# xipengwang/AprilSAM

Hardware: NVIDIA H100
Metric: Gauss-Newton solves/sec (batch + incremental) on M3500 & 100k-pose graph (higher is better)
Workload: dtype f64

## Files before the change

### aprilsam_b200/csrc/asam_cuda.cu

```cuda

#include <cuda_runtime.h>

#include <cmath>
#include <cstdarg>
#include <cstdint>
#include <cstdio>
#include <cstdlib>
#include <cstring>
#include <ctime>

#include "asam_cuda.h"

#define ASAM_EXPORT extern "C" __attribute__((visibility("default")))

static thread_local char g_err[512] = "";

static int set_err(const char *fmt, ...)
{
    va_list ap;
    va_start(ap, fmt);
    vsnprintf(g_err, sizeof(g_err), fmt, ap);
    va_end(ap);
    return 1;
}
// ... 527 lines not shown
        const int v = atoi(getenv("ASAM_DIAG_MMA")) != 0;
        CK(cudaMemcpyToSymbol(g_diag_mma, &v, sizeof(int)));
    }
    if (getenv("ASAM_DMAP_AHEAD")) {
        const int v = atoi(getenv("ASAM_DMAP_AHEAD")) != 0;
        CK(cudaMemcpyToSymbol(g_dmap_ahead, &v, sizeof(int)));
    }
    if (getenv("ASAM_PF_GROUPS")) {
        const int v = atoi(getenv("ASAM_PF_GROUPS")) != 0;
        CK(cudaMemcpyToSymbol(g_pf_groups, &v, sizeof(int)));
    }
    if (getenv("ASAM_KEEP"))
        d->keep_off = atoi(getenv("ASAM_KEEP")) == 0;
    if (getenv("ASAM_TILE_MODE"))
        d->tile_mode = atoi(getenv("ASAM_TILE_MODE"));
    if (getenv("ASAM_SMALL_STEP"))
        d->small_ok = atoi(getenv("ASAM_SMALL_STEP")) != 0;
    memset(d->pin_down, 0, 64);
    *out = d;
    return 0;
}

ASAM_EXPORT void asam_dev_destroy(asam_dev_t *d)
{
    if (!d)
        return;
    cudaSetDevice(d->device);
    cudaStreamSynchronize(d->stream);
    Buf *all[] = { &d->f_type, &d->f_a, &d->f_b, &d->f_z, &d->f_W, &d->f_slot, &d->lp, &d->st, &d->node2q, &d->q2node,
                   &d->Adiag, &d->Aoff, &d->Bq, &d->y, &d->x, &d->dinv, &d->sn, &d->ipool, &d->arena, &d->arrive,
                   &d->xdone, &d->xblk, &d->tbar, &d->tasks_full, &d->nwait_full, &d->btasks_full, &d->tasks_tmp, &d->nwait_tmp,
                   &d->btasks_tmp, &d->keep_tmp, &d->leaf_tasks, &d->top_tasks, &d->top_nwait, &d->ctrl, &d->partial, &d->patch_ids, &d->patch_desc, &d->pts, &d->flush, &d->trace_fac, &d->trace_bs, &d->ptrace };
    for (int i = 0; i < 2; i++)
        if (d->tev[i])
            cudaEventDestroy(d->tev[i]);
    for (Buf *b : all)
        if (b->p)
            cudaFree(b->p);
    if (d->pin)
        cudaFreeHost(d->pin);
    if (d->pin_down)
        cudaFreeHost(d->pin_down);
    if (d->dstage)
        cudaFree(d->dstage);
    if (d->up_ev)
        cudaEventDestroy(d->up_ev);
    free(d->items);
    free(d->pend);
    free(d->sh_owner); free(d->sh_q0); free(d->sh_qn); free(d->sh_off); free(d->sh_cnt);
    for (int i = 0; i < 6; i++)
        if (d->ev[i])
            cudaEventDestroy(d->ev[i]);
    cudaStreamDestroy(d->stream);
    delete d;
}

ASAM_EXPORT int asam_reserve(asam_dev_t *d, int n_nodes, int n_factors, int n_slots, int n_sn, int64_t ipool_ints,
                             int64_t arena_doubles)
{
    CK(cudaSetDevice(d->device));
    size_t N = (size_t) (n_nodes > 0 ? n_nodes : 0), Fn = (size_t) (n_factors > 0 ? n_factors : 0);
    size_t S = (size_t) (n_slots > 0 ? n_slots : 0), SN = (size_t) (n_sn > 0 ? n_sn : 0);
    int rc = 0;
    rc |= buf_reserve(d, d->f_type, Fn * sizeof(int), true, false);
    rc |= buf_reserve(d, d->f_a, Fn * sizeof(int), true, false);
    rc |= buf_reserve(d, d->f_b, Fn * sizeof(int), true, false);
    rc |= buf_reserve(d, d->f_slot, Fn * sizeof(int), true, false);
    rc |= buf_reserve(d, d->f_z, Fn * 3 * sizeof(double), true, false);
    rc |= buf_reserve(d, d->f_W, Fn * 9 * sizeof(double), true, false);
    rc |= buf_reserve(d, d->lp, N * 3 * sizeof(double), true, false);
    rc |= buf_reserve(d, d->st, N * 3 * sizeof(double), true, false);
    rc |= buf_reserve(d, d->node2q, N * sizeof(int), true, false);
    rc |= buf_reserve(d, d->q2node, N * sizeof(int), true, false);
    rc |= buf_reserve(d, d->Adiag, N * 9 * sizeof(double), true, true);
    rc |= buf_reserve(d, d->Bq, N * 3 * sizeof(double), true, true);
    rc |= buf_reserve(d, d->y, N * 3 * sizeof(double), true, true);
    rc |= buf_reserve(d, d->x, N * 3 * sizeof(double), true, true);
    rc |= buf_reserve(d, d->dinv, N * 3 * sizeof(double), true, true);
    rc |= buf_reserve(d, d->Aoff, S * 9 * sizeof(double), true, true);
    rc |= buf_reserve(d, d->sn, SN * sizeof(asam_sn_desc_t), true, false);
    rc |= buf_reserve(d, d->arrive, SN * sizeof(int), true, true);
    rc |= buf_reserve(d, d->xdone, SN * sizeof(int), true, true);
    rc |= buf_reserve(d, d->xblk, SN * sizeof(int), true, true);
    rc |= buf_reserve(d, d->tbar, 2 * SN * sizeof(int), true, true);
    rc |= buf_reserve(d, d->ipool, (size_t) ipool_ints * sizeof(int), true, false);
    rc |= buf_reserve(d, d->arena, (size_t) arena_doubles * sizeof(double), true, false);
    return rc;
}

ASAM_EXPORT int asam_upload_factors(asam_dev_t *d, int first, int count, const int32_t *type, const int32_t *na,
                                    const int32_t *nb, const double *z3, const double *W9)
{
    if (count <= 0)
        return 0;
    size_t need = (size_t) first + count;
    if (need * sizeof(int) > d->f_type.cap)
        return set_err("asam_upload_factors: capacity (call asam_reserve)");
    int rc = 0;
    rc |= upload(d, (int *) d->f_type.p + first, type, count * sizeof(int));
    rc |= upload(d, (int *) d->f_a.p + first, na, count * sizeof(int));
    rc |= upload(d, (int *) d->f_b.p + first, nb, count * sizeof(int));
    rc |= upload(d, (double *) d->f_z.p + 3 * (size_t) first, z3, count * 3 * sizeof(double));
    rc |= upload(d, (double *) d->f_W.p + 9 * (size_t) first, W9, count * 9 * sizeof(double));
    return rc;
}

ASAM_EXPORT int asam_upload_points(asam_dev_t *d, int which, int first, int count, const double *p3)
{
    if (count <= 0)
        return 0;
    Buf &b = which == 0 ? d->lp : d->st;
    if (((size_t) first + count) * 3 * sizeof(double) > b.cap)
        return set_err("asam_upload_points: capacity");
    return upload(d, (double *) b.p + 3 * (size_t) first, p3, (size_t) count * 3 * sizeof(double));
}

ASAM_EXPORT int asam_copy_points(asam_dev_t *d, int from, int to, int first, int count)
{
    if (count <= 0 || from == to)
        return 0;
    CK(cudaSetDevice(d->device));
    Buf &src = from == 0 ? d->lp : d->st, &dst = to == 0 ? d->lp : d->st;
    const size_t off = (size_t) first * 3 * sizeof(double), bytes = (size_t) count * 3 * sizeof(double);
    if (off + bytes > src.cap || off + bytes > dst.cap)
        return set_err("asam_copy_points: capacity");
    if (flush_uploads(d))
        return 1;
    CK(cudaMemcpyAsync((char *) dst.p + off, (const char *) src.p + off, bytes, cudaMemcpyDeviceToDevice, d->stream));
    return 0;
}

ASAM_EXPORT int asam_upload_node2q(asam_dev_t *d, int first, int count, const int32_t *node2q)
{
    if (count <= 0)
        return 0;
    if (((size_t) first + count) * sizeof(int) > d->node2q.cap)
        return set_err("asam_upload_node2q: capacity");
    return upload(d, (int *) d->node2q.p + first, node2q, (size_t) count * sizeof(int));
}

ASAM_EXPORT int asam_upload_q2node(asam_dev_t *d, int first, int count, const int32_t *q2node)
{
    if (count <= 0)
        return 0;
    if (((size_t) first + count) * sizeof(int) > d->q2node.cap)
        return set_err("asam_upload_q2node: capacity");
    return upload(d, (int *) d->q2node.p + first, q2node, (size_t) count * sizeof(int));
}

ASAM_EXPORT int asam_upload_fslot(asam_dev_t *d, int first, int count, const int32_t *fslot)
{
    if (count <= 0)
        return 0;
    if (((size_t) first + count) * sizeof(int) > d->f_slot.cap)
        return set_err("asam_upload_fslot: capacity");
    return upload(d, (int *) d->f_slot.p + first, fslot, (size_t) count * sizeof(int));
}

ASAM_EXPORT int asam_upload_ipool(asam_dev_t *d, int64_t first, int64_t count, const int32_t *data)
{
    if (count <= 0)
        return 0;
    if ((size_t) (first + count) * sizeof(int) > d->ipool.cap)
        return set_err("asam_upload_ipool: capacity");
    return upload(d, (int *) d->ipool.p + first, data, (size_t) count * sizeof(int));
}

// ... 852 lines not shown
```

### aprilsam_b200/csrc/asam_kernels.cuh

```cuda
#pragma once

#include <cuda_runtime.h>

#include <cstdint>

#include "asam_cuda.h"

#define ASAM_TR_FLAG (1 << 30)
#define ASAM_MAX_CACHED_CHILDREN 24

__device__ __forceinline__ double d_mod2pi(double v)
{
    const double twopi = 6.2831853071795862319959;
    const double pi = 3.141592653589793238462643383279502884196;
    double w = v + pi;
    return (w - twopi * floor(w / twopi)) - pi;
}

__device__ __forceinline__ void d_atb(const double *A, const double *B, double *C)
{
#pragma unroll
    for (int i = 0; i < 3; i++)
#pragma unroll
        for (int j = 0; j < 3; j++) {
// ... 525 lines not shown
                bulk_g2s(Lj + (size_t) p * ASAM_LDJ, col + (cb0 - shj), bj, bar);
            }
        }
        for (int e = tid; e < (pb4 - pb) * ASAM_LDI; e += nt)
            Li[(size_t) pb * ASAM_LDI + e] = 0.0;
        for (int e = tid; e < (pb4 - pb) * ASAM_LDJ; e += nt)
            Lj[(size_t) pb * ASAM_LDJ + e] = 0.0;
    } else {
        for (int p = warp; p < pb4; p += 2 * nwarps) {
            double vj[2][2], vi[2][8];
#pragma unroll
            for (int h = 0; h < 2; h++) {
                const int pp = p + h * nwarps;
                const double *src = F + (size_t) (k0 + min(pp, pb - 1)) * ld;
#pragma unroll
                for (int u = 0; u < 2; u++)
                    vj[h][u] = (pp < pb && lane + 32 * u < ncol) ? __ldcg(src + cb0 + lane + 32 * u) : 0.0;
#pragma unroll
                for (int u = 0; u < 8; u++)
                    vi[h][u] = (pp < pb && lane + 32 * u < nrow) ? __ldcg(src + rb0 + lane + 32 * u) : 0.0;
            }
#pragma unroll
            for (int h = 0; h < 2; h++) {
                const int pp = p + h * nwarps;
                if (pp < pb4) {
#pragma unroll
                    for (int u = 0; u < 2; u++)
                        Lj[lane + 32 * u + pp * ASAM_LDJ] = vj[h][u];
#pragma unroll
                    for (int u = 0; u < 8; u++)
                        Li[lane + 32 * u + pp * ASAM_LDI] = vi[h][u];
                }
            }
        }
    }
    const int g = lane >> 2, t = lane & 3;
    const int r0 = warp * 8 * MT;
    const int nnt = (ncol + 7) >> 3;
    const int rowmax = rb0 + min(r0 + 8 * MT, nrow) - 1;
    const int nneed = (r0 < nrow && rowmax >= cb0) ? min(nnt, ((rowmax - cb0) >> 3) + 1) : 0;
    double acc[MT][8][2];
#pragma unroll
    for (int mt = 0; mt < MT; mt++)
#pragma unroll
        for (int q = 0; q < 8; q++)
#pragma unroll
            for (int e = 0; e < 2; e++) {
                const int ii = r0 + 8 * mt + g, jj = 8 * q + 2 * t + e;
                const bool ok = q < nneed && ii < nrow && jj < ncol && rb0 + ii >= cb0 + jj;
                acc[mt][q][e] = ok ? __ldcg(&F[(rb0 + ii) + (size_t) (cb0 + jj) * ld]) : 0.0;
            }
    if (bulk) {
        mbar_wait(bar, parity);
        parity ^= 1u;
    }
    __syncthreads();
    if (nneed > 0) {
        const double *ai = Li + shi + r0 + g + (size_t) t * ASAM_LDI;
        const double *bj_ = Lj + shj + g + (size_t) t * ASAM_LDJ;
#pragma unroll 2
        for (int kk = 0; kk < pb4; kk += 4) {
            double av[MT];
#pragma unroll
            for (int mt = 0; mt < MT; mt++)
                av[mt] = -ai[8 * mt + (size_t) kk * ASAM_LDI];
#pragma unroll
            for (int q = 0; q < 8; q++) {
                if (q < nneed) {
                    const double bv = bj_[8 * q + (size_t) kk * ASAM_LDJ];
#pragma unroll
                    for (int mt = 0; mt < MT; mt++)
                        dmma_8x8x4(acc[mt][q][0], acc[mt][q][1], av[mt], bv);
                }
            }
        }
#pragma unroll
        for (int mt = 0; mt < MT; mt++)
#pragma unroll
            for (int q = 0; q < 8; q++)
#pragma unroll
                for (int e = 0; e < 2; e++) {
                    const int ii = r0 + 8 * mt + g, jj = 8 * q + 2 * t + e;
                    if (q < nneed && ii < nrow && jj < ncol && rb0 + ii >= cb0 + jj) {
                        F[(rb0 + ii) + (size_t) (cb0 + jj) * ld] = acc[mt][q][e];
                        if (Dout)
                            Dout[ii + jj * ASAM_TPB] = acc[mt][q][e];
                    }
                }
    }
}

#define ASAM_LDW 52
#define ASAM_WS_DOUBLES(m) (2 * (size_t) ((m) + 2) * ASAM_LDW)

template <int MT>
__device__ __noinline__ void tile_rm(double *F, const int ld, const double *Wk, const int pb4, const int cb0, const int ncol,
                                     const int rb0, const int nrow, const int out_mode, double *Out, double *Li, double *Lj,
                                     unsigned long long *bar, unsigned &parity)
{
    const int tid = threadIdx.x;
    const int lane = tid & 31, warp = tid >> 5;
    const bool same = rb0 == cb0 && nrow >= ncol;
    __syncthreads();
    if (warp == 0) {
        asm volatile("fence.proxy.async;" ::: "memory");
        if (lane == 0) {
            const unsigned bi = (unsigned) nrow * ASAM_LDW * 8u, bj = same ? 0u : (unsigned) ncol * ASAM_LDW * 8u;
            mbar_expect_tx(bar, bi + bj);
            bulk_g2s(Li, Wk + (size_t) rb0 * ASAM_LDW, bi, bar);
            if (!same)
                bulk_g2s(Lj, Wk + (size_t) cb0 * ASAM_LDW, bj, bar);
        }
    }
    const double *Ljs = same ? Li : Lj;
    const int g = lane >> 2, t = lane & 3;
    const int r0 = warp * 8 * MT;
    const int nnt = (ncol + 7) >> 3;
    const int rowmax = rb0 + min(r0 + 8 * MT, nrow) - 1;
    const int nneed = (r0 < nrow && rowmax >= cb0) ? min(nnt, ((rowmax - cb0) >> 3) + 1) : 0;
    double acc[MT][8][2];
#pragma unroll
    for (int mt = 0; mt < MT; mt++)
#pragma unroll
        for (int q = 0; q < 8; q++)
#pragma unroll
            for (int e = 0; e < 2; e++) {
                const int ii = r0 + 8 * mt + g, jj = 8 * q + 2 * t + e;
                const bool ok = q < nneed && ii < nrow && jj < ncol && rb0 + ii >= cb0 + jj;
                acc[mt][q][e] = ok ? __ldcg(&F[(rb0 + ii) + (size_t) (cb0 + jj) * ld]) : 0.0;
            }
    mbar_wait(bar, parity);
    parity ^= 1u;
    if (nneed > 0) {
        const double *ai = Li + (size_t) (r0 + g) * ASAM_LDW + t;
        const double *bj_ = Ljs + (size_t) g * ASAM_LDW + t;
#pragma unroll 2
        for (int kk = 0; kk < pb4; kk += 4) {
            double av[MT];
#pragma unroll
            for (int mt = 0; mt < MT; mt++)
                av[mt] = -ai[(size_t) (8 * mt) * ASAM_LDW + kk];
#pragma unroll
            for (int q = 0; q < 8; q++) {
                if (q < nneed) {
                    const double bv = bj_[(size_t) (8 * q) * ASAM_LDW + kk];
#pragma unroll
                    for (int mt = 0; mt < MT; mt++)
                        dmma_8x8x4(acc[mt][q][0], acc[mt][q][1], av[mt], bv);
                }
            }
        }
    }
    if (out_mode == 2)
        __syncthreads();
    if (nneed > 0) {
#pragma unroll
        for (int mt = 0; mt < MT; mt++)
#pragma unroll
            for (int q = 0; q < 8; q++)
#pragma unroll
                for (int e = 0; e < 2; e++) {
                    const int ii = r0 + 8 * mt + g, jj = 8 * q + 2 * t + e;
                    if (q < nneed && ii < nrow && jj < ncol && rb0 + ii >= cb0 + jj) {
                        if (out_mode == 0)
                            F[(rb0 + ii) + (size_t) (cb0 + jj) * ld] = acc[mt][q][e];
                        else if (out_mode == 1)
                            Out[ii + jj * ASAM_TPB] = acc[mt][q][e];
                        else
                            Out[ii + jj * ASAM_TROWS] = acc[mt][q][e];
                    }
                }
    }
}

struct TeamCtx {
    int *tbar_s;
    int G, w, phase;
    long long spin_limit;
    int *err;
    int sn;
};

__device__ __forceinline__ bool team_barrier(TeamCtx &tc, int *s_flag)
{
    __syncthreads();
    if (threadIdx.x == 0) {
        red_release_add(tc.tbar_s, 1);
        const int target = (++tc.phase) * tc.G;
        SpinClock spins;
        int ok = 1;
        while (ld_volatile(tc.tbar_s) < target) {
            __nanosleep(20);
            if (spin_over(spins, tc.spin_limit) || ld_volatile(tc.err) < 0) {
                atomicCAS(tc.err, 0, -(1 + tc.sn));
                ok = 0;
                break;
            }
        }
        ld_acquire(tc.tbar_s);
        *s_flag = ok;
    } else {
        tc.phase++;
    }
    __syncthreads();
    return *s_flag != 0;
}

__device__ __forceinline__ void team_leave(TeamCtx &tc)
{
    if (threadIdx.x == 0) {
        const int v = atomicAdd(tc.tbar_s, 1);
        if (v == tc.phase * tc.G + tc.G - 1)
            atomicExch(tc.tbar_s, 0);
    }
}

__device__ __forceinline__ bool team_owns(int col, int w, int G) { return ((col >> 2) % G) == w; }

__device__ __forceinline__ void diag_factor(double *D, int pb, double *rdv, int sn_id, int *err)
{
    const int tid = threadIdx.x;
    constexpr int LDD = ASAM_TPB;
    for (int c0 = 0; c0 < pb; c0 += 3) {
        if (c0 > 0 && tid < 3 * (pb - c0)) {
            const int i = c0 + tid / 3, j = c0 + tid % 3;
            if (i >= j) {
                double acc0 = D[i + j * LDD], acc1 = 0.0;
                int p = 0;
                for (; p + 1 < c0; p += 2) {
                    acc0 -= D[i + p * LDD] * D[j + p * LDD];
                    acc1 -= D[i + (p + 1) * LDD] * D[j + (p + 1) * LDD];
                }
                if (p < c0)
                    acc0 -= D[i + p * LDD] * D[j + p * LDD];
                D[i + j * LDD] = acc0 + acc1;
            }
        }
        __syncthreads();
        double *p0 = D + c0 * LDD, *p1 = p0 + LDD, *p2 = p1 + LDD;
        const double a00 = p0[c0], a10 = p0[c0 + 1], a20 = p0[c0 + 2];
        const double a11 = p1[c0 + 1], a21 = p1[c0 + 2], a22 = p2[c0 + 2];
        const double r0 = d_rsqrt(a00);
        const double l10 = a10 * r0, l20 = a20 * r0;
        const double d1 = a11 - l10 * l10;
        const double r1 = d_rsqrt(d1);
        const double l21 = (a21 - l20 * l10) * r1;
        const double d2 = a22 - l20 * l20 - l21 * l21;
        const double r2 = d_rsqrt(d2);
        if (tid == 0 && !(a00 > 0.0 && d1 > 0.0 && d2 > 0.0))
            atomicCAS(err, 0, 1 + sn_id);
        const int i = c0 + 3 + tid;
        if (i < pb) {
            const double x0 = p0[i] * r0;
            const double x1 = (p1[i] - x0 * l10) * r1;
            const double x2 = (p2[i] - x0 * l20 - x1 * l21) * r2;
            p0[i] = x0;
            p1[i] = x1;
            p2[i] = x2;
        }
        __syncthreads();
        if (tid == 0) {
            p0[c0] = a00 * r0; p0[c0 + 1] = l10; p0[c0 + 2] = l20;
            p1[c0 + 1] = d1 * r1; p1[c0 + 2] = l21;
            p2[c0 + 2] = d2 * r2;
            rdv[c0] = r0; rdv[c0 + 1] = r1; rdv[c0 + 2] = r2;
        }
    }
    __syncthreads();
}

__device__ __forceinline__ void diag_factor_rl(double *D, int pb, double *rdv, int sn_id, int *err)
{
    constexpr int LDD = ASAM_TPB;
    constexpr int SUB = 256;
    if (threadIdx.x < SUB) {
        for (int k1 = 0; k1 < pb; k1 += ASAM_PB) {
            const int pbb = min(ASAM_PB, pb - k1);
            panel_factor(D + (size_t) k1 * LDD, LDD, k1, pbb, pb - 1, sn_id, err, rdv, SUB);
            if (k1 + pbb < pb) {
                if (g_diag_mma)
                    trailing_update_mma(D, LDD, D + (size_t) k1 * LDD, LDD, pbb, k1 + pbb, pb, pb - 1, SUB / 32);
                else
                    trailing_update<1, 4>(D, LDD, D + (size_t) k1 * LDD, LDD, pbb, k1 + pbb, pb, pb - 1, SUB / 32);
                bar_sub(SUB);
            }
        }
    }
    __syncthreads();
}

__device__ __forceinline__ void trsm_row_block(double *Li, const double *D, const double *rdv, const int b0, const int nb,
                                               double *Frow, int ld, double *Wrow)
{
    const int tid = threadIdx.x;
    constexpr int LDD = ASAM_TPB;
    double r[12];
#pragma unroll
    for (int q = 0; q < 12; q++)
        r[q] = (q < nb) ? Li[tid + (b0 + q) * ASAM_TROWS] : 0.0;
    for (int p = 0; p < b0; p++) {
        const double xp = Li[tid + p * ASAM_TROWS];
        const double2 *Dp = reinterpret_cast<const double2 *>(D + p * LDD + b0);
#pragma unroll
        for (int q2 = 0; q2 < 6; q2++) {
            const double2 v = Dp[q2];
            r[2 * q2] -= xp * v.x;
            r[2 * q2 + 1] -= xp * v.y;
        }
    }
#pragma unroll
    for (int q = 0; q < 12; q++) {
        if (q < nb) {
            r[q] *= rdv[b0 + q];
#pragma unroll
            for (int q2 = q + 1; q2 < 12; q2++)
                r[q2] -= r[q] * D[(b0 + q2) + (b0 + q) * LDD];
        }
    }
#pragma unroll
    for (int q = 0; q < 12; q++)
        if (q < nb) {
            Li[tid + (b0 + q) * ASAM_TROWS] = r[q];
            Frow[(size_t) (b0 + q) * ld] = r[q];
            if (Wrow)
                Wrow[b0 + q] = r[q];
        }
}

__device__ __forceinline__ void trsm_row(double *Li, const double *D, const double *rdv, int pb, double *Frow, int ld,
                                         double *Wrow = nullptr)
{
    for (int b0 = 0; b0 < pb; b0 += 12)
        trsm_row_block(Li, D, rdv, b0, min(12, pb - b0), Frow, ld, Wrow);
    if (Wrow)
        for (int q = pb; q < ((pb + 3) & ~3); q++)
            Wrow[q] = 0.0;
}

__device__ bool team_front(const FacArgs &a, const asam_sn_desc_t &d, int s, int nw, int w, int G, double *sm,
                           int *s_flag, unsigned long long *trow, unsigned long long *mbar, unsigned &mb_parity)
{
    const int tid = threadIdx.x, nt = blockDim.x;
    const int lane = tid & 31, warp = tid >> 5, nwarps = nt >> 5;
    const int m = 3 * d.mb, c = 3 * d.cb, ld = ASAM_LD(m);
    const int *seg = a.ipool + d.seg;
    const int *children = seg + 2 * d.mb;
    const int *a_slot = children + d.ch_cnt;
    const int *a_rb = a_slot + d.a_cnt;
    const int *a_cb = a_rb + d.a_cnt;
    double *F = a.arena + d.f_off;
    int *err = a.ctrl + 1;
    TeamCtx tc;
    tc.tbar_s = a.tbar + 2 * (size_t) s;
    tc.G = G;
    tc.w = w;
    tc.phase = 0;
    tc.spin_limit = a.spin_limit;
    tc.err = err;
    tc.sn = s;

    for (int j = warp; j < m; j += nwarps) {
        if (!team_owns(j, w, G))
            continue;
        for (int i = j + lane; i <= m; i += 32)
            F[i + (size_t) j * ld] = 0.0;
    }
    __syncthreads();
    for (int e = tid; e < d.cb * 9; e += nt) {
        int k = e / 9, p = (e % 9) / 3, q = e % 3;
        if (p >= q && team_owns(3 * k + q, w, G))
            F[(3 * k + p) + (size_t) (3 * k + q) * ld] = a.Adiag[9 * (size_t) a.q2node[d.first + k] + q * 3 + p];
    }
    for (int e = tid; e < c; e += nt)
        if (team_owns(e, w, G))
            F[m + (size_t) e * ld] = a.Bq[3 * (size_t) a.q2node[d.first + e / 3] + e % 3];
    for (int e = tid; e < d.a_cnt * 9; e += nt) {
        int i = e / 9, p = (e % 9) / 3, q = e % 3;
        const int col = 3 * a_cb[i] + q;
        if (!team_owns(col, w, G))
            continue;
        const int rbf = a_rb[i];
        const int rb = rbf & ~ASAM_TR_FLAG;
        const int si = (rbf & ASAM_TR_FLAG) ? (p * 3 + q) : (q * 3 + p);
        F[(3 * rb + p) + (size_t) col * ld] = a.Aoff[9 * (size_t) a_slot[i] + si];
    }
    if (nw > 0 && tid == 0) {
        SpinClock spins;
        int ok = 1;
        while (ld_volatile(&a.arrive[s]) < nw) {
            __nanosleep(20);
            if (spin_over(spins, a.spin_limit) || ld_volatile(err) < 0) {
                atomicCAS(err, 0, -(1 + s));
                ok = 0;
                break;
            }
        }
        __threadfence();
        *s_flag = ok;
    } else if (tid == 0) {
        *s_flag = 1;
    }
    __syncthreads();
    if (!*s_flag)
        return false;
    if (trow && tid == 0)
        trow[1] = trow[2] = d_now();

    int *dmap = (int *) sm;
    for (int ci = 0; ci < d.ch_cnt; ++ci) {
        const asam_sn_desc_t cd = a.sn[children[ci]];
        const int cm = 3 * cd.mb, cc = 3 * cd.cb, cr = cm - cc, cld = ASAM_LD(cm);
        const double *CF = a.arena + cd.f_off;
        const int *crel = a.ipool + cd.seg + cd.mb;
        __syncthreads();
        for (int i = tid; i <= cr; i += nt)
            dmap[i] = (i < cr) ? 3 * crel[(cc + i) / 3] + (cc + i) % 3 : m;
        __syncthreads();
        for (int j = warp; j < cr; j += nwarps) {
            const int dj = dmap[j];
            if (!team_owns(dj, w, G))
                continue;
            const double *ccol = CF + (size_t) (cc + j) * cld + cc;
            double *fcol = F + (size_t) dj * ld;
            for (int i0 = j + lane; i0 <= cr; i0 += 256) {
                double v[8], dv[8];
                int di[8];
#pragma unroll
                for (int u = 0; u < 8; u++) {
                    const bool ok = i0 + 32 * u <= cr;
                    v[u] = ok ? __ldcg(ccol + i0 + 32 * u) : 0.0;
                    di[u] = ok ? dmap[i0 + 32 * u] : -1;
                }
#pragma unroll
                for (int u = 0; u < 8; u++)
                    dv[u] = di[u] >= 0 ? __ldcg(fcol + di[u]) : 0.0;
#pragma unroll
                for (int u = 0; u < 8; u++)
                    if (di[u] >= 0)
                        fcol[di[u]] = dv[u] + v[u];
            }
        }
    }
    if (!team_barrier(tc, s_flag))
        return false;
    if (w == 0 && nw > 0 && tid == 0)
        a.arrive[s] = 0;
    unsigned long long t_panel = 0, t_mark = 0;
    if (trow && tid == 0)
        trow[3] = d_now();

    double *D = sm;
    double *rdv = D + ASAM_TPB * ASAM_TPB;
    double *Li = rdv + ASAM_TPB;
    double *Lj = Li + ASAM_LDI * ASAM_TPB;
    const bool v3 = a.tile_mode == 3;
    double *Wbase = F + (size_t) ld * m;
    auto Wbuf = [&](int panel_index) { return Wbase + (size_t) (panel_index & 1) * (m + 2) * ASAM_LDW; };
    double *Lj3 = Li + ASAM_TROWS * ASAM_LDW;
    double *dinv = a.dinv + 3 * (size_t) d.first;
    int *crew_bar = a.tbar + 2 * (size_t) s + 1;

    auto tile = [&](int k0, int pb, int cb0, int ncol, int rb0, int nrow, double *Dout) {
        if (v3) {
            const double *Wk = Wbuf(k0 / ASAM_TPB);
            const int pb4 = (pb + 3) & ~3;
            if (Dout)
                tile_rm<1>(F, ld, Wk, pb4, cb0, ncol, rb0, nrow, 1, Dout, Li, Lj3, mbar, mb_parity);
            else if (nrow <= 128)
                tile_rm<2>(F, ld, Wk, pb4, cb0, ncol, rb0, nrow, 0, nullptr, Li, Lj3, mbar, mb_parity);
            else
                tile_rm<4>(F, ld, Wk, pb4, cb0, ncol, rb0, nrow, 0, nullptr, Li, Lj3, mbar, mb_parity);
            return;
        }
        if (a.tile_mode != 0) {
            const int bulk = a.tile_mode == 2;
            if (nrow <= 64)
                tile_mma<1>(F, ld, m, k0, pb, cb0, ncol, rb0, nrow, Dout, Li, Lj, mbar, mb_parity, bulk);
            else if (nrow <= 128)
                tile_mma<2>(F, ld, m, k0, pb, cb0, ncol, rb0, nrow, Dout, Li, Lj, mbar, mb_parity, bulk);
            else
                tile_mma<4>(F, ld, m, k0, pb, cb0, ncol, rb0, nrow, Dout, Li, Lj, mbar, mb_parity, bulk);
            return;
        }
        __syncthreads();
        for (int p = warp; p < pb; p += 2 * nwarps) {
            double vj[2][2], vi[2][8];
#pragma unroll
            for (int h = 0; h < 2; h++) {
                const int pp = p + h * nwarps;
                const double *src = F + (size_t) (k0 + min(pp, pb - 1)) * ld;
#pragma unroll
                for (int u = 0; u < 2; u++)
                    vj[h][u] = (pp < pb && lane + 32 * u < ncol) ? __ldcg(src + cb0 + lane + 32 * u) : 0.0;
#pragma unroll
                for (int u = 0; u < 8; u++)
                    vi[h][u] = (pp < pb && lane + 32 * u < nrow) ? __ldcg(src + rb0 + lane + 32 * u) : 0.0;
            }
#pragma unroll
            for (int h = 0; h < 2; h++) {
                const int pp = p + h * nwarps;
                if (pp < pb) {
#pragma unroll
                    for (int u = 0; u < 2; u++)
                        if (lane + 32 * u < ncol)
                            Lj[lane + 32 * u + pp * ASAM_TCOLS] = vj[h][u];
#pragma unroll
                    for (int u = 0; u < 8; u++)
                        if (lane + 32 * u < nrow)
                            Li[lane + 32 * u + pp * ASAM_TROWS] = vi[h][u];
                }
            }
        }
        __syncthreads();
        const int tj = 8 * warp;
        if (tj < ncol) {
            for (int ib = 0; ib < nrow; ib += 128) {
                double acc[4][8], cv[4][8];
                int ir[4], jc[8];
#pragma unroll
                for (int q = 0; q < 8; q++)
                    jc[q] = min(tj + q, ncol - 1);
#pragma unroll
                for (int r = 0; r < 4; r++) {
                    ir[r] = min(ib + lane + 32 * r, nrow - 1);
#pragma unroll
                    for (int q = 0; q < 8; q++) {
                        acc[r][q] = 0.0;
                        const int ii = ib + lane + 32 * r, jj = tj + q;
                        const bool ok = ii < nrow && jj < ncol && rb0 + ii >= cb0 + jj;
                        cv[r][q] = ok ? __ldcg(&F[(rb0 + ii) + (size_t) (cb0 + jj) * ld]) : 0.0;
                    }
                }
#pragma unroll 2
                for (int p = 0; p < pb; p++) {
                    double bq[8], av[4];
#pragma unroll
                    for (int q = 0; q < 8; q++)
                        bq[q] = Lj[jc[q] + p * ASAM_TCOLS];
#pragma unroll
                    for (int r = 0; r < 4; r++)
                        av[r] = Li[ir[r] + p * ASAM_TROWS];
#pragma unroll
                    for (int r = 0; r < 4; r++)
#pragma unroll
                        for (int q = 0; q < 8; q++)
                            acc[r][q] += av[r] * bq[q];
                }
#pragma unroll
                for (int r = 0; r < 4; r++)
#pragma unroll
                    for (int q = 0; q < 8; q++) {
                        const int ii = ib + lane + 32 * r, jj = tj + q;
                        const int i = rb0 + ii, j = cb0 + jj;
                        if (ii < nrow && jj < ncol && i >= j) {
                            const double v = cv[r][q] - acc[r][q];
                            F[i + (size_t) j * ld] = v;
                            if (Dout)
                                Dout[ii + jj * ASAM_TPB] = v;
                        }
                    }
            }
        }
    };
    auto panel = [&](int k0, int pb, int rb0) {
        __syncthreads();
        for (int e = tid; e < ASAM_TPB * ASAM_TPB; e += nt) {
            const int i = e % ASAM_TPB, j = e / ASAM_TPB;
            D[e] = (i >= j && i < pb && j < pb) ? __ldcg(&F[(k0 + i) + (size_t) (k0 + j) * ld]) : 0.0;
        }
        const int i = rb0 + tid;
        const bool row = rb0 >= 0 && i >= k0 + pb && i <= m;
        if (row)
            for (int j = 0; j < pb; j++)
                Li[tid + j * ASAM_TROWS] = __ldcg(&F[i + (size_t) (k0 + j) * ld]);
        __syncthreads();
        if (v3)
            diag_factor_rl(D, pb, rdv, s, err);
        else
            diag_factor(D, pb, rdv, s, err);
        if (row)
            trsm_row(Li, D, rdv, pb, F + i + (size_t) k0 * ld, ld, v3 ? Wbuf(0) + (size_t) i * ASAM_LDW : nullptr);
    };
    auto writeback = [&](int k0, int pb) {
        for (int e = tid; e < pb * pb; e += nt) {
            const int i = e % pb, j = e / pb;
            if (i >= j)
                F[(k0 + i) + (size_t) (k0 + j) * ld] = D[i + j * ASAM_TPB];
        }
        for (int e = tid; e < pb; e += nt)
            dinv[k0 + e] = rdv[e];
    };

    auto diag_publish = [&](int k0, int pb, int seq) {
        __syncthreads();
        if (v3) {
            constexpr int LDD = ASAM_TPB;
            constexpr int SUB = 256;
            int stage = 0;
            for (int k1 = 0; k1 < pb; k1 += ASAM_PB) {
                const int pbb = min(ASAM_PB, pb - k1);
                panel_factor(D + (size_t) k1 * LDD, LDD, k1, pbb, pb - 1, s, err, rdv, SUB);
                ++stage;
                for (int e = tid; e < pbb * pb; e += SUB) {
                    const int j = k1 + e / pb, i = e % pb;
                    if (i >= j)
                        F[(k0 + i) + (size_t) (k0 + j) * ld] = D[i + j * LDD];
                }
                for (int e = tid; e < pbb; e += SUB)
                    dinv[k0 + k1 + e] = rdv[k1 + e];
                bar_sub(SUB);
                if (tid == 0)
                    st_release(crew_bar, 8 * seq + stage);
                if (k1 + pbb < pb) {
                    if (g_diag_mma)
                        trailing_update_mma(D, LDD, D + (size_t) k1 * LDD, LDD, pbb, k1 + pbb, pb, pb - 1, SUB / 32);
                    else
                        trailing_update<1, 4>(D, LDD, D + (size_t) k1 * LDD, LDD, pbb, k1 + pbb, pb, pb - 1, SUB / 32);
                    bar_sub(SUB);
                }
            }
            __syncthreads();
            return;
        }
        diag_factor(D, pb, rdv, s, err);
        writeback(k0, pb);
        __syncthreads();
        if (tid == 0) {
            __threadfence();
            atomicExch(crew_bar, seq);
        }
    };
    auto rows_solve_staged = [&](int k0, int pb, int rb0, int seq, double *Wnext) {
        constexpr int LDD = ASAM_TPB;
        if (tid == 0)
            *s_flag = 1;
        __syncthreads();
        const int i = rb0 + tid;
        const bool row = tid < ASAM_CROWS && i <= m;
        int stage = 0;
        for (int b0 = 0; b0 < pb; b0 += ASAM_PB, ++stage) {
            const int nb = min(ASAM_PB, pb - b0);
            if (warp >= 4) {
                if (tid == 128 && *s_flag) {
                    SpinClock spins;
                    while (ld_volatile(crew_bar) < 8 * seq + stage + 1) {
                        __nanosleep(20);
                        if (spin_over(spins, a.spin_limit) || ld_volatile(err) < 0) {
                            atomicCAS(err, 0, -(1 + s));
                            *s_flag = 0;
                            break;
                        }
                    }
                    ld_acquire(crew_bar);
                }
                asm volatile("bar.sync 2, 128;" ::: "memory");
                if (*s_flag) {
                    for (int e = tid - 128; e < nb * ASAM_TPB; e += 128) {
                        const int j = b0 + e / ASAM_TPB, ii = e % ASAM_TPB;
                        D[ii + j * LDD] = (ii >= j && ii < pb) ? __ldcg(&F[(k0 + ii) + (size_t) (k0 + j) * ld]) : 0.0;
                    }
                    if (tid - 128 < nb)
                        rdv[b0 + tid - 128] = __ldcg(&dinv[k0 + b0 + tid - 128]);
                }
                __threadfence_block();
                asm volatile("bar.arrive %0, 256;" ::"r"(3 + stage) : "memory");
            } else {
                asm volatile("bar.sync %0, 256;" ::"r"(3 + stage) : "memory");
                if (row && *s_flag)
                    trsm_row_block(Li, D, rdv, b0, nb, F + i + (size_t) k0 * ld, ld, Wnext + (size_t) i * ASAM_LDW);
            }
        }
        if (row && *s_flag)
            for (int q = pb; q < ((pb + 3) & ~3); q++)
                Wnext[(size_t) i * ASAM_LDW + q] = 0.0;
        __syncthreads();
        return *s_flag != 0;
    };
    auto rows_solve = [&](int k0, int pb, int rb0, int seq, double *Wnext) {
        __syncthreads();
        const int i = rb0 + tid;
        const bool row = tid < ASAM_CROWS && i <= m;
        if (row && !Wnext)
            for (int j = 0; j < pb; j++)
                Li[tid + j * ASAM_TROWS] = __ldcg(&F[i + (size_t) (k0 + j) * ld]);
        if (tid == 0) {
            SpinClock spins;
            int ok = 1;
            while (ld_volatile(crew_bar) < seq) {
                __nanosleep(20);
                if (spin_over(spins, a.spin_limit) || ld_volatile(err) < 0) {
                    atomicCAS(err, 0, -(1 + s));
                    ok = 0;
                    break;
                }
            }
            __threadfence();
            *s_flag = ok;
        }
        __syncthreads();
        if (!*s_flag)
            return false;
        for (int e = tid; e < ASAM_TPB * ASAM_TPB; e += nt) {
            const int ii = e % ASAM_TPB, j = e / ASAM_TPB;
            D[e] = (ii >= j && ii < pb && j < pb) ? __ldcg(&F[(k0 + ii) + (size_t) (k0 + j) * ld]) : 0.0;
        }
        for (int e = tid; e < ASAM_TPB; e += nt)
            rdv[e] = e < pb ? __ldcg(&dinv[k0 + e]) : 0.0;
        __syncthreads();
        if (row)
            trsm_row(Li, D, rdv, pb, F + i + (size_t) k0 * ld, ld, Wnext ? Wnext + (size_t) i * ASAM_LDW : nullptr);
        return true;
    };

    {
        const int pb = min(ASAM_TPB, c);
        if (trow && tid == 0)
            t_mark = d_now();
        const int nchunk = (m + 1 + ASAM_TROWS - 1) / ASAM_TROWS;
        bool first = true;
        for (int ch = w; ch < nchunk || first; ch += G) {
            panel(0, pb, ch < nchunk ? ch * ASAM_TROWS : -1);
            first = false;
        }
        if (!team_barrier(tc, s_flag))
            return false;
        if (trow && tid == 0)
            t_panel += d_now() - t_mark;
        if (w == 0)
            writeback(0, pb);
    }
    int seq = 0;
    const bool pt_on = a.ptrace && s == a.ptrace_sn && w < 8 && tid == 0;
    for (int k0 = 0; k0 < c; k0 += ASAM_TPB) {
        unsigned long long *pt = (pt_on && k0 / ASAM_TPB < a.ptrace_panels) ? a.ptrace + ((size_t) (k0 / ASAM_TPB) * 8 + w) * 8 : nullptr;
        if (pt) {
            pt[0] = d_now();
            pt[1] = pt[2] = pt[3] = pt[0];
            pt[5] = (unsigned long long) m;
            pt[6] = (unsigned long long) G;
        }
        const int pb = min(ASAM_TPB, c - k0);
        const int kn0 = k0 + pb;
        const bool has_next = kn0 < c;
        const int pbn = has_next ? min(ASAM_TPB, c - kn0) : 0;
        const int ncrew = has_next ? 1 + (m - (kn0 + pbn) + 1 + ASAM_CROWS - 1) / ASAM_CROWS : 0;
        ++seq;
        if (w < ncrew) {
            if (trow && tid == 0)
                t_mark = d_now();
            if (w == 0) {
                __syncthreads();
                for (int e = tid; e < ASAM_TPB * ASAM_TPB; e += nt)
                    D[e] = 0.0;
                tile(k0, pb, kn0, pbn, kn0, pbn, D);
                if (pt)
                    pt[1] = d_now();
                diag_publish(kn0, pbn, seq);
                if (pt)
                    pt[2] = d_now();
            }
            if (v3) {
                for (int it = (w == 0 ? G : w); it < ncrew; it += G) {
                    const int rb0 = kn0 + pbn + (it - 1) * ASAM_CROWS;
                    tile_rm<2>(F, ld, Wbuf(k0 / ASAM_TPB), (pb + 3) & ~3, kn0, pbn, rb0, min(ASAM_CROWS, m - rb0 + 1), 2, Li, Li,
                               Lj3, mbar, mb_parity);
                    if (pt && w > 0 && it == w)
                        pt[1] = d_now();
                    if (!rows_solve_staged(kn0, pbn, rb0, seq, Wbuf(kn0 / ASAM_TPB)))
                        return false;
                }
            } else {
                for (int it = (w == 0 ? G : w); it < ncrew; it += G) {
                    const int rb0 = kn0 + pbn + (it - 1) * ASAM_CROWS;
                    tile(k0, pb, kn0, pbn, rb0, min(ASAM_CROWS, m - rb0 + 1), nullptr);
                }
                if (pt && w > 0)
                    pt[1] = d_now();
                for (int it = (w == 0 ? G : w); it < ncrew; it += G) {
                    const int rb0 = kn0 + pbn + (it - 1) * ASAM_CROWS;
                    if (!rows_solve(kn0, pbn, rb0, seq, nullptr))
                        return false;
                }
            }
            if (pt && w > 0)
                pt[2] = d_now();
            if (trow && tid == 0)
                t_panel += d_now() - t_mark;
        }

        const int j0 = kn0 + pbn;
        const int nfree = (G - ncrew >= 2) ? G - ncrew : G, wfree = (G - ncrew >= 2) ? w - ncrew : w;
        int n256 = 0;
        for (int cb0 = j0; cb0 < m; cb0 += ASAM_TCOLS)
            n256 += (m - cb0 + 1 + 255) / 256;
        const int TR = (n256 < 2 * nfree) ? 128 : 256;
        if (wfree >= 0) {
            int u = 0;
            for (int cb0 = j0; cb0 < m; cb0 += ASAM_TCOLS)
                for (int rb0 = cb0; rb0 <= m; rb0 += TR, ++u)
                    if (u % nfree == wfree)
                        tile(k0, pb, cb0, min(ASAM_TCOLS, m - cb0), rb0, min(TR, m - rb0 + 1), nullptr);
        }
        if (pt)
            pt[3] = d_now();
        if (!team_barrier(tc, s_flag))
            return false;
        if (pt) {
            pt[4] = d_now();
            pt[7] = (unsigned long long) ncrew;
        }
    }
    if (w == 0 && tid == 0)
        atomicExch(crew_bar, 0);

    if (trow && tid == 0) {
        trow[4] = d_now();
        trow[7] = (unsigned long long) (unsigned) m | (t_panel << 32);
    }
    if (w == 0) {
        for (int e = tid; e < c; e += nt)
            a.y[3 * (size_t) d.first + e] = __ldcg(&F[m + (size_t) e * ld]);
        __syncthreads();
        if (tid == 0 && d.parent >= 0) {
            __threadfence();
            atomicAdd(&a.arrive[d.parent], 1);
        }
    }
    team_leave(tc);
    __syncthreads();
    return true;
}

__device__ __forceinline__ void ticket_release(int *ticket, int *done)
{
    __syncthreads();
    if (threadIdx.x == 0) {
        __threadfence();
        if (atomicAdd(done, 1) == (int) gridDim.x - 1) {
            atomicExch(ticket, 0);
            atomicExch(done, 0);
        }
    }
}

__device__ bool cta_front(const FacArgs &a, const int t, const int s, const int nw, const asam_sn_desc_t &d, double *sm,
                          asam_sn_desc_t *s_cd, int *s_abort, unsigned long long tr0, const int keepw = 0)
{
    const int tid = threadIdx.x, nt = blockDim.x;
    const int lane = tid & 31, warp = tid >> 5, nwarps = nt >> 5;
    int *err = a.ctrl + 1;
    unsigned long long tr1 = 0, tr2 = 0, tr3 = 0, tr4 = 0, accA = 0, accB = 0;
    const int m = 3 * d.mb, c = 3 * d.cb, ld = ASAM_LD(m);
    const int *seg = a.ipool + d.seg;
    const int *children = seg + 2 * d.mb;
    const int *a_slot = children + d.ch_cnt;
    const int *a_rb = a_slot + d.a_cnt;
    const int *a_cb = a_rb + d.a_cnt;
    double *Fg = a.arena + d.f_off;
    const long long fsz = (long long) ld * m;
    const bool use_sm = fsz + (ld + 1) / 2 + 2 <= (long long) a.smem_doubles;
    double *F = use_sm ? sm : Fg;
    int *dmap = (int *) (sm + (use_sm ? fsz : 0));
    double *Pbuf = sm + (ld + 1) / 2 + 1;
    double *dinv = a.dinv + 3 * (size_t) d.first;

    if (use_sm) {
        for (int i = tid; i < (int) fsz; i += nt)
            F[i] = 0.0;
    } else {
        for (int j = warp; j < m; j += nwarps)
            for (int i = j + lane; i <= m; i += 32)
                F[i + (size_t) j * ld] = 0.0;
    }
    for (int e = tid; e < d.ch_cnt && e < ASAM_MAX_CACHED_CHILDREN; e += nt)
        s_cd[e] = a.sn[children[e]];
    __syncthreads();
    __shared__ int s_doff[ASAM_MAX_CACHED_CHILDREN + 1];
    bool dmap_ahead = false;
    if (use_sm && g_dmap_ahead && d.ch_cnt > 0 && d.ch_cnt <= ASAM_MAX_CACHED_CHILDREN) {
        if (tid == 0) {
            int o = 0;
            for (int e = 0; e < d.ch_cnt; e++) {
                s_doff[e] = o;
                o += 3 * (s_cd[e].mb - s_cd[e].cb) + 1;
            }
            s_doff[d.ch_cnt] = o;
        }
        __syncthreads();
        dmap_ahead = (long long) s_doff[d.ch_cnt] <= 2 * ((long long) a.smem_doubles - fsz) - 2;
        if (dmap_ahead)
            for (int ci = 0; ci < d.ch_cnt; ++ci) {
                const int cc = 3 * s_cd[ci].cb, cr = 3 * s_cd[ci].mb - cc;
                const int *crel = a.ipool + s_cd[ci].seg + s_cd[ci].mb;
                int *dm = dmap + s_doff[ci];
                for (int i = tid; i <= cr; i += nt)
                    dm[i] = (i < cr) ? 3 * crel[(cc + i) / 3] + (cc + i) % 3 : m;
// ... 1030 lines not shown
```

Before: 128.3.

## Factor diagonal redundantly per crew block, removing cross-block crew barrier

Every crew block now computes the next diagonal tile itself and factors it locally. Inside a block, warp-specialized named barriers let 128 threads factor the diagonal while the other 128 load their row chunk and run the triangular solve stage by stage. This replaces the global-memory crew_bar publish/spin handshake in which block 0 factored and wrote back before the other blocks could proceed. Writeback of the diagonal moves to the start of the next panel, and diagonal tiles are no longer written to F in the tile kernels. The cost is redundant diagonal factorization in every crew block and more complex barrier choreography.

```diff
diff --git a/aprilsam_b200/csrc/asam_cuda.cu b/aprilsam_b200/csrc/asam_cuda.cu
--- a/aprilsam_b200/csrc/asam_cuda.cu
+++ b/aprilsam_b200/csrc/asam_cuda.cu
@@ -633,7 +633,7 @@
     rc |= buf_reserve(d, d->arrive, SN * sizeof(int), true, true);
     rc |= buf_reserve(d, d->xdone, SN * sizeof(int), true, true);
     rc |= buf_reserve(d, d->xblk, SN * sizeof(int), true, true);
-    rc |= buf_reserve(d, d->tbar, 2 * SN * sizeof(int), true, true);
+    rc |= buf_reserve(d, d->tbar, SN * sizeof(int), true, true);
     rc |= buf_reserve(d, d->ipool, (size_t) ipool_ints * sizeof(int), true, false);
     rc |= buf_reserve(d, d->arena, (size_t) arena_doubles * sizeof(double), true, false);
     return rc;
diff --git a/aprilsam_b200/csrc/asam_kernels.cuh b/aprilsam_b200/csrc/asam_kernels.cuh
--- a/aprilsam_b200/csrc/asam_kernels.cuh
+++ b/aprilsam_b200/csrc/asam_kernels.cuh
@@ -631,9 +631,10 @@
                 for (int e = 0; e < 2; e++) {
                     const int ii = r0 + 8 * mt + g, jj = 8 * q + 2 * t + e;
                     if (q < nneed && ii < nrow && jj < ncol && rb0 + ii >= cb0 + jj) {
-                        F[(rb0 + ii) + (size_t) (cb0 + jj) * ld] = acc[mt][q][e];
                         if (Dout)
                             Dout[ii + jj * ASAM_TPB] = acc[mt][q][e];
+                        else
+                            F[(rb0 + ii) + (size_t) (cb0 + jj) * ld] = acc[mt][q][e];
                     }
                 }
     }
@@ -642,16 +643,25 @@
 #define ASAM_LDW 52
 #define ASAM_WS_DOUBLES(m) (2 * (size_t) ((m) + 2) * ASAM_LDW)
 
-template <int MT>
+template <int MT, int GROUP = -1>
 __device__ __noinline__ void tile_rm(double *F, const int ld, const double *Wk, const int pb4, const int cb0, const int ncol,
                                      const int rb0, const int nrow, const int out_mode, double *Out, double *Li, double *Lj,
                                      unsigned long long *bar, unsigned &parity)
 {
     const int tid = threadIdx.x;
-    const int lane = tid & 31, warp = tid >> 5;
+    const int lane = tid & 31, warp = (tid >> 5) - (GROUP == 1 ? 4 : 0);
+    auto sync = [] {
+        if (GROUP == 0)
+            asm volatile("bar.sync 1, 128;" ::: "memory");
+        else if (GROUP == 1)
+            asm volatile("bar.sync 2, 128;" ::: "memory");
+        else
+            __syncthreads();
+    };
     const bool same = rb0 == cb0 && nrow >= ncol;
-    __syncthreads();
-    if (warp == 0) {
+    if (GROUP < 0)
+        sync();
+    if (GROUP < 0 && warp == 0) {
         asm volatile("fence.proxy.async;" ::: "memory");
         if (lane == 0) {
             const unsigned bi = (unsigned) nrow * ASAM_LDW * 8u, bj = same ? 0u : (unsigned) ncol * ASAM_LDW * 8u;
@@ -701,7 +711,7 @@
         }
     }
     if (out_mode == 2)
-        __syncthreads();
+        sync();
     if (nneed > 0) {
 #pragma unroll
         for (int mt = 0; mt < MT; mt++)
@@ -838,10 +848,9 @@
     __syncthreads();
 }
 
-__device__ __forceinline__ void trsm_row_block(double *Li, const double *D, const double *rdv, const int b0, const int nb,
-                                               double *Frow, int ld, double *Wrow)
-{
-    const int tid = threadIdx.x;
+__device__ __forceinline__ void trsm_row_block(double *Li, const int tid, const double *D, const double *rdv, const int b0,
+                                               const int nb, double *Frow, int ld, double *Wrow)
+{
     constexpr int LDD = ASAM_TPB;
     double r[12];
 #pragma unroll
@@ -880,10 +889,51 @@
                                          double *Wrow = nullptr)
 {
     for (int b0 = 0; b0 < pb; b0 += 12)
-        trsm_row_block(Li, D, rdv, b0, min(12, pb - b0), Frow, ld, Wrow);
+        trsm_row_block(Li, threadIdx.x, D, rdv, b0, min(12, pb - b0), Frow, ld, Wrow);
     if (Wrow)
         for (int q = pb; q < ((pb + 3) & ~3); q++)
             Wrow[q] = 0.0;
+}
+
+template <class FillBlock, class FillRows>
+__device__ __forceinline__ void diag_factor_rows(double *D, const int pb, double *rdv, const int sn_id, int *err, double *Li,
+                                                 const int nrow, double *Frow, const int ld, double *Wrow, FillBlock fill_block,
+                                                 FillRows fill_rows)
+{
+    constexpr int LDD = ASAM_TPB;
+    constexpr int NF = 128;
+    const int tid = threadIdx.x;
+    __syncthreads();
+    if (tid < NF) {
+        fill_block();
+        int stage = 0;
+        for (int k1 = 0; k1 < pb; k1 += ASAM_PB, ++stage) {
+            const int pbb = min(ASAM_PB, pb - k1);
+            panel_factor(D + (size_t) k1 * LDD, LDD, k1, pbb, pb - 1, sn_id, err, rdv, NF);
+            __threadfence_block();
+            asm volatile("bar.arrive %0, 256;" ::"r"(3 + stage) : "memory");
+            if (k1 + pbb < pb) {
+                if (g_diag_mma)
+                    trailing_update_mma(D, LDD, D + (size_t) k1 * LDD, LDD, pbb, k1 + pbb, pb, pb - 1, NF / 32);
+                else
+                    trailing_update<1, 4>(D, LDD, D + (size_t) k1 * LDD, LDD, pbb, k1 + pbb, pb, pb - 1, NF / 32);
+                bar_sub(NF);
+            }
+        }
+    } else {
+        const int r = tid - NF;
+        fill_rows();
+        int stage = 0;
+        for (int b0 = 0; b0 < pb; b0 += ASAM_PB, ++stage) {
+            asm volatile("bar.sync %0, 256;" ::"r"(3 + stage) : "memory");
+            if (r < nrow)
+                trsm_row_block(Li, r, D, rdv, b0, min(ASAM_PB, pb - b0), Frow + r, ld, Wrow + (size_t) r * ASAM_LDW);
+        }
+        if (r < nrow)
+            for (int q = pb; q < ((pb + 3) & ~3); q++)
+                Wrow[(size_t) r * ASAM_LDW + q] = 0.0;
+    }
+    __syncthreads();
 }
 
 __device__ bool team_front(const FacArgs &a, const asam_sn_desc_t &d, int s, int nw, int w, int G, double *sm,
@@ -900,7 +950,7 @@
     double *F = a.arena + d.f_off;
     int *err = a.ctrl + 1;
     TeamCtx tc;
-    tc.tbar_s = a.tbar + 2 * (size_t) s;
+    tc.tbar_s = a.tbar + s;
     tc.G = G;
     tc.w = w;
     tc.phase = 0;
@@ -1007,7 +1057,6 @@
     auto Wbuf = [&](int panel_index) { return Wbase + (size_t) (panel_index & 1) * (m + 2) * ASAM_LDW; };
     double *Lj3 = Li + ASAM_TROWS * ASAM_LDW;
     double *dinv = a.dinv + 3 * (size_t) d.first;
-    int *crew_bar = a.tbar + 2 * (size_t) s + 1;
 
     auto tile = [&](int k0, int pb, int cb0, int ncol, int rb0, int nrow, double *Dout) {
         if (v3) {
@@ -1103,9 +1152,10 @@
                         const int i = rb0 + ii, j = cb0 + jj;
                         if (ii < nrow && jj < ncol && i >= j) {
                             const double v = cv[r][q] - acc[r][q];
-                            F[i + (size_t) j * ld] = v;
                             if (Dout)
                                 Dout[ii + jj * ASAM_TPB] = v;
+                            else
+                                F[i + (size_t) j * ld] = v;
                         }
                     }
             }
@@ -1140,127 +1190,6 @@
             dinv[k0 + e] = rdv[e];
     };
 
-    auto diag_publish = [&](int k0, int pb, int seq) {
-        __syncthreads();
-        if (v3) {
-            constexpr int LDD = ASAM_TPB;
-            constexpr int SUB = 256;
-            int stage = 0;
-            for (int k1 = 0; k1 < pb; k1 += ASAM_PB) {
-                const int pbb = min(ASAM_PB, pb - k1);
-                panel_factor(D + (size_t) k1 * LDD, LDD, k1, pbb, pb - 1, s, err, rdv, SUB);
-                ++stage;
-                for (int e = tid; e < pbb * pb; e += SUB) {
-                    const int j = k1 + e / pb, i = e % pb;
-                    if (i >= j)
-                        F[(k0 + i) + (size_t) (k0 + j) * ld] = D[i + j * LDD];
-                }
-                for (int e = tid; e < pbb; e += SUB)
-                    dinv[k0 + k1 + e] = rdv[k1 + e];
-                bar_sub(SUB);
-                if (tid == 0)
-                    st_release(crew_bar, 8 * seq + stage);
-                if (k1 + pbb < pb) {
-                    if (g_diag_mma)
-                        trailing_update_mma(D, LDD, D + (size_t) k1 * LDD, LDD, pbb, k1 + pbb, pb, pb - 1, SUB / 32);
-                    else
-                        trailing_update<1, 4>(D, LDD, D + (size_t) k1 * LDD, LDD, pbb, k1 + pbb, pb, pb - 1, SUB / 32);
-                    bar_sub(SUB);
-                }
-            }
-            __syncthreads();
-            return;
-        }
-        diag_factor(D, pb, rdv, s, err);
-        writeback(k0, pb);
-        __syncthreads();
-        if (tid == 0) {
-            __threadfence();
-            atomicExch(crew_bar, seq);
-        }
-    };
-    auto rows_solve_staged = [&](int k0, int pb, int rb0, int seq, double *Wnext) {
-        constexpr int LDD = ASAM_TPB;
-        if (tid == 0)
-            *s_flag = 1;
-        __syncthreads();
-        const int i = rb0 + tid;
-        const bool row = tid < ASAM_CROWS && i <= m;
-        int stage = 0;
-        for (int b0 = 0; b0 < pb; b0 += ASAM_PB, ++stage) {
-            const int nb = min(ASAM_PB, pb - b0);
-            if (warp >= 4) {
-                if (tid == 128 && *s_flag) {
-                    SpinClock spins;
-                    while (ld_volatile(crew_bar) < 8 * seq + stage + 1) {
-                        __nanosleep(20);
-                        if (spin_over(spins, a.spin_limit) || ld_volatile(err) < 0) {
-                            atomicCAS(err, 0, -(1 + s));
-                            *s_flag = 0;
-                            break;
-                        }
-                    }
-                    ld_acquire(crew_bar);
-                }
-                asm volatile("bar.sync 2, 128;" ::: "memory");
-                if (*s_flag) {
-                    for (int e = tid - 128; e < nb * ASAM_TPB; e += 128) {
-                        const int j = b0 + e / ASAM_TPB, ii = e % ASAM_TPB;
-                        D[ii + j * LDD] = (ii >= j && ii < pb) ? __ldcg(&F[(k0 + ii) + (size_t) (k0 + j) * ld]) : 0.0;
-                    }
-                    if (tid - 128 < nb)
-                        rdv[b0 + tid - 128] = __ldcg(&dinv[k0 + b0 + tid - 128]);
-                }
-                __threadfence_block();
-                asm volatile("bar.arrive %0, 256;" ::"r"(3 + stage) : "memory");
-            } else {
-                asm volatile("bar.sync %0, 256;" ::"r"(3 + stage) : "memory");
-                if (row && *s_flag)
-                    trsm_row_block(Li, D, rdv, b0, nb, F + i + (size_t) k0 * ld, ld, Wnext + (size_t) i * ASAM_LDW);
-            }
-        }
-        if (row && *s_flag)
-            for (int q = pb; q < ((pb + 3) & ~3); q++)
-                Wnext[(size_t) i * ASAM_LDW + q] = 0.0;
-        __syncthreads();
-        return *s_flag != 0;
-    };
-    auto rows_solve = [&](int k0, int pb, int rb0, int seq, double *Wnext) {
-        __syncthreads();
-        const int i = rb0 + tid;
-        const bool row = tid < ASAM_CROWS && i <= m;
-        if (row && !Wnext)
-            for (int j = 0; j < pb; j++)
-                Li[tid + j * ASAM_TROWS] = __ldcg(&F[i + (size_t) (k0 + j) * ld]);
-        if (tid == 0) {
-            SpinClock spins;
-            int ok = 1;
-            while (ld_volatile(crew_bar) < seq) {
-                __nanosleep(20);
-                if (spin_over(spins, a.spin_limit) || ld_volatile(err) < 0) {
-                    atomicCAS(err, 0, -(1 + s));
-                    ok = 0;
-                    break;
-                }
-            }
-            __threadfence();
-            *s_flag = ok;
-        }
-        __syncthreads();
-        if (!*s_flag)
-            return false;
-        for (int e = tid; e < ASAM_TPB * ASAM_TPB; e += nt) {
-            const int ii = e % ASAM_TPB, j = e / ASAM_TPB;
-            D[e] = (ii >= j && ii < pb && j < pb) ? __ldcg(&F[(k0 + ii) + (size_t) (k0 + j) * ld]) : 0.0;
-        }
-        for (int e = tid; e < ASAM_TPB; e += nt)
-            rdv[e] = e < pb ? __ldcg(&dinv[k0 + e]) : 0.0;
-        __syncthreads();
-        if (row)
-            trsm_row(Li, D, rdv, pb, F + i + (size_t) k0 * ld, ld, Wnext ? Wnext + (size_t) i * ASAM_LDW : nullptr);
-        return true;
-    };
-
     {
         const int pb = min(ASAM_TPB, c);
         if (trow && tid == 0)
@@ -1275,12 +1204,12 @@
             return false;
         if (trow && tid == 0)
             t_panel += d_now() - t_mark;
-        if (w == 0)
-            writeback(0, pb);
-    }
-    int seq = 0;
+    }
     const bool pt_on = a.ptrace && s == a.ptrace_sn && w < 8 && tid == 0;
     for (int k0 = 0; k0 < c; k0 += ASAM_TPB) {
+        const int pb = min(ASAM_TPB, c - k0);
+        if (w == 0)
+            writeback(k0, pb);
         unsigned long long *pt = (pt_on && k0 / ASAM_TPB < a.ptrace_panels) ? a.ptrace + ((size_t) (k0 / ASAM_TPB) * 8 + w) * 8 : nullptr;
         if (pt) {
             pt[0] = d_now();
@@ -1288,50 +1217,72 @@
             pt[5] = (unsigned long long) m;
             pt[6] = (unsigned long long) G;
         }
-        const int pb = min(ASAM_TPB, c - k0);
         const int kn0 = k0 + pb;
         const bool has_next = kn0 < c;
         const int pbn = has_next ? min(ASAM_TPB, c - kn0) : 0;
         const int ncrew = has_next ? 1 + (m - (kn0 + pbn) + 1 + ASAM_CROWS - 1) / ASAM_CROWS : 0;
-        ++seq;
         if (w < ncrew) {
             if (trow && tid == 0)
                 t_mark = d_now();
-            if (w == 0) {
-                __syncthreads();
-                for (int e = tid; e < ASAM_TPB * ASAM_TPB; e += nt)
-                    D[e] = 0.0;
+            const int it0 = w == 0 ? G : w;
+            auto chunk_row = [&](int it) { return kn0 + pbn + (it - 1) * ASAM_CROWS; };
+            auto chunk_rows = [&](int it) { return it < ncrew ? min(ASAM_CROWS, m - chunk_row(it) + 1) : 0; };
+            __syncthreads();
+            for (int e = tid; e < ASAM_TPB * ASAM_TPB; e += nt)
+                D[e] = 0.0;
+            if (v3) {
+                const double *Wk = Wbuf(k0 / ASAM_TPB);
+                double *Wn = Wbuf(kn0 / ASAM_TPB);
+                double *Xb = Lj3 + ASAM_TCOLS * ASAM_LDW;
+                const int pb4 = (pb + 3) & ~3;
+                const int nr0 = chunk_rows(it0), rb00 = chunk_row(it0);
+                if (warp == 0) {
+                    asm volatile("fence.proxy.async;" ::: "memory");
+                    if (lane == 0) {
+                        const unsigned bb = (unsigned) pbn * ASAM_LDW * 8u, br = (unsigned) nr0 * ASAM_LDW * 8u;
+                        mbar_expect_tx(mbar, bb + br);
+                        bulk_g2s(Xb, Wk + (size_t) kn0 * ASAM_LDW, bb, mbar);
+                        if (nr0 > 0)
+                            bulk_g2s(Li, Wk + (size_t) rb00 * ASAM_LDW, br, mbar);
+                    }
+                }
+                diag_factor_rows(
+                    D, pbn, rdv, s, err, Li, nr0, F + rb00 + (size_t) kn0 * ld, ld, Wn + (size_t) rb00 * ASAM_LDW,
+                    [&] {
+                        tile_rm<2, 0>(F, ld, Wk, pb4, kn0, pbn, kn0, pbn, 1, D, Xb, Xb, mbar, mb_parity);
+                        if (pt)
+                            pt[1] = d_now();
+                    },
+                    [&] {
+                        if (nr0 > 0)
+                            tile_rm<4, 1>(F, ld, Wk, pb4, kn0, pbn, rb00, nr0, 2, Li, Li, Xb, mbar, mb_parity);
+                        else
+                            mb_parity ^= 1u;
+                    });
+                for (int it = it0 + G; it < ncrew; it += G) {
+                    const int rb0 = chunk_row(it), nr = chunk_rows(it);
+                    tile_rm<2>(F, ld, Wk, pb4, kn0, pbn, rb0, nr, 2, Li, Li, Lj3, mbar, mb_parity);
+                    __syncthreads();
+                    if (tid < nr)
+                        trsm_row(Li, D, rdv, pbn, F + rb0 + tid + (size_t) kn0 * ld, ld, Wn + (size_t) (rb0 + tid) * ASAM_LDW);
+                }
+            } else {
                 tile(k0, pb, kn0, pbn, kn0, pbn, D);
+                for (int it = it0; it < ncrew; it += G)
+                    tile(k0, pb, kn0, pbn, chunk_row(it), chunk_rows(it), nullptr);
                 if (pt)
                     pt[1] = d_now();
-                diag_publish(kn0, pbn, seq);
-                if (pt)
-                    pt[2] = d_now();
-            }
-            if (v3) {
-                for (int it = (w == 0 ? G : w); it < ncrew; it += G) {
-                    const int rb0 = kn0 + pbn + (it - 1) * ASAM_CROWS;
-                    tile_rm<2>(F, ld, Wbuf(k0 / ASAM_TPB), (pb + 3) & ~3, kn0, pbn, rb0, min(ASAM_CROWS, m - rb0 + 1), 2, Li, Li,
-                               Lj3, mbar, mb_parity);
-                    if (pt && w > 0 && it == w)
-                        pt[1] = d_now();
-                    if (!rows_solve_staged(kn0, pbn, rb0, seq, Wbuf(kn0 / ASAM_TPB)))
-                        return false;
-                }
-            } else {
-                for (int it = (w == 0 ? G : w); it < ncrew; it += G) {
-                    const int rb0 = kn0 + pbn + (it - 1) * ASAM_CROWS;
-                    tile(k0, pb, kn0, pbn, rb0, min(ASAM_CROWS, m - rb0 + 1), nullptr);
-                }
-                if (pt && w > 0)
-                    pt[1] = d_now();
-                for (int it = (w == 0 ? G : w); it < ncrew; it += G) {
-                    const int rb0 = kn0 + pbn + (it - 1) * ASAM_CROWS;
-                    if (!rows_solve(kn0, pbn, rb0, seq, nullptr))
-                        return false;
-                }
-            }
-            if (pt && w > 0)
+                diag_factor(D, pbn, rdv, s, err);
+                for (int it = it0; it < ncrew; it += G) {
+                    const int i = chunk_row(it) + tid;
+                    if (tid < chunk_rows(it)) {
+                        for (int j = 0; j < pbn; j++)
+                            Li[tid + j * ASAM_TROWS] = __ldcg(&F[i + (size_t) (kn0 + j) * ld]);
+                        trsm_row(Li, D, rdv, pbn, F + i + (size_t) kn0 * ld, ld);
+                    }
+                }
+            }
+            if (pt)
                 pt[2] = d_now();
             if (trow && tid == 0)
                 t_panel += d_now() - t_mark;
@@ -1359,8 +1310,6 @@
             pt[7] = (unsigned long long) ncrew;
         }
     }
-    if (w == 0 && tid == 0)
-        atomicExch(crew_bar, 0);
 
     if (trow && tid == 0) {
         trow[4] = d_now();
```

Result: no change. 128.5 (median of 6 runs) (+0.2%).
